# tusen-ai/SST

Measured on AMD Instinct MI355X. Metric: LiDAR frames/sec (SST backbone fwd+bwd) at Waymo 0.32m voxels, higher is better.
Workload: dtype f32 (storage, accumulation, attention, LayerNorm, reductions: fp32; the dense products of the encoder layers from the EXACT three-way bf16 split of both fp32 operands, six bf16 MFMA products with fp32 accumulation - error vs float64 <= 2 x the fp32 matrix pipe's: tests/test_gpu_dense_f32x6.py)

## Files before the change

include/sst_amd.h:

```cpp
#ifndef SST_AMD_H
#define SST_AMD_H

#include <stdint.h>

#ifdef __cplusplus
extern "C" {
#endif

#define SST_OK 0
#define SST_ERR_ARG (-1)
#define SST_ERR_UNSUPPORTED (-2)
#define SST_ERR_KEYSPACE (-3)

typedef enum { SST_REDUCE_SUM = 0, SST_REDUCE_MEAN = 1, SST_REDUCE_MAX = 2 } sst_reduce_t;

const char* sst_version(void);

int sst_dynamic_voxelize_f32(const float* d_points, int64_t n, int64_t row_stride,
                             const float voxel_size[3], const float coors_range[6],
                             int32_t* d_coors, int64_t coors_stride, int coors_col0, int batch_idx,
                             void* stream);
void sst_dynamic_voxelize_grid(const float voxel_size[3], const float coors_range[6], int32_t grid_xyz[3]);

int64_t sst_scan_workspace_bytes(int64_t n);
// ... 184 lines not shown
int sst_add_layernorm_act_bwd_f32(const float* d_dy, const float* d_sum, const float* d_stats, const float* d_weight,
                                  const float* d_bias, int act, int64_t m, int c, float* d_dx, float* d_dweight,
                                  float* d_dbias, void* d_workspace, void* stream);
int sst_add_layernorm_fwd_f32(const float* d_x, const float* d_res, const float* d_weight, const float* d_bias,
                              int64_t m, int c, float eps, float* d_y, float* d_sum, float* d_stats,
                              void* stream);
int sst_add_layernorm_pos_fwd_f32(const float* d_x, const float* d_res, const float* d_weight, const float* d_bias, int64_t m,
                                  int c, float eps, float* d_y, float* d_sum, float* d_stats, const float* d_pos_table,
                                  const int32_t* d_pos_idx, float* d_y_plus_pos, void* stream);
int64_t sst_add_layernorm_bwd_workspace_bytes(int64_t m, int c);
int sst_add_layernorm_bwd_f32(const float* d_dy, const float* d_sum, const float* d_stats,
                              const float* d_weight, int64_t m, int c, float* d_dx, float* d_dweight,
                              float* d_dbias, void* d_workspace, void* stream);
int64_t sst_colsum_workspace_bytes(int64_t m, int c);
int sst_colsum_f32(const float* d_x, int64_t m, int c, int64_t ld, float* d_out, void* d_workspace, void* stream);

int64_t sst_weight_grad_workspace_bytes(int64_t m, int out, int in);
int sst_weight_grad_f32(const float* d_dy, const float* d_x, int64_t m, int out, int in, int64_t ld_dy,
                        int64_t ld_x, float* d_dw, float* d_db, void* d_workspace, void* stream);
typedef struct sst_wgrad_problem_f32 {
  const float* dy;
  const float* x;
  int64_t m, ld_dy, ld_x;
  float* dw;
  float* db;
  int32_t out, in;
  const float* x_add_rows;
  const int32_t* x_add_index;
} sst_wgrad_problem_f32;
int64_t sst_weight_grad_group_workspace_bytes(const sst_wgrad_problem_f32* problems, int n);
int sst_weight_grad_group_f32(const sst_wgrad_problem_f32* problems, int n, void* d_workspace, void* stream);
int64_t sst_weight_grad_group_f32x6_workspace_bytes(const sst_wgrad_problem_f32* problems, int n);
int sst_weight_grad_group_f32x6(const sst_wgrad_problem_f32* problems, int n, void* d_workspace, void* stream);

int64_t sst_bn_workspace_bytes(int64_t n, int c);
int sst_bn_stats_f32(const float* d_x, int64_t n, int c, int64_t ld, float* d_mean, float* d_var,
                     void* d_workspace, void* stream);
int sst_bn_act_fwd_f32(const float* d_x, int64_t n, int c, int64_t ldx, const float* d_scale,
                       const float* d_shift, int act, float* d_y, int64_t ldy, void* stream);
int sst_bn_act_bwd_reduce_f32(const float* d_dy, const float* d_x, int64_t n, int c, int64_t lddy, int64_t ldx,
                              const float* d_mean, const float* d_invstd, const float* d_scale,
                              const float* d_shift, int act, float* d_sum_g, float* d_sum_gxhat,
                              void* d_workspace, void* stream);
int sst_bn_act_bwd_apply_f32(const float* d_dy, const float* d_x, int64_t n, int c, int64_t lddy, int64_t ldx,
                             const float* d_mean, const float* d_invstd, const float* d_scale,
                             const float* d_shift, const float* d_coef_a, const float* d_coef_b, float coef_scale,
                             int act, float* d_dx, int64_t lddx, void* stream);
int sst_bn_prepare_f32(const float* d_x, int64_t n, int c, int64_t ld, const float* d_weight, const float* d_bias,
                       float eps, float* d_running_mean, float* d_running_var, float factor, float* d_out4,
                       void* d_workspace, void* stream);
int sst_bn_prepare_tracked_f32(const float* d_x, int64_t n, int c, int64_t ld, const float* d_weight,
                               const float* d_bias, float eps, float* d_running_mean, float* d_running_var,
                               float factor, int64_t* d_num_batches_tracked, float* d_out4, void* d_workspace,
                               void* stream);
int sst_vfe_linear_moments_f32(const float* d_x, int64_t ldx, int64_t n, int k, const float* d_w, int64_t ldw, int c,
                               float* d_y, int64_t ldy, void* d_workspace, void* stream);
int sst_bn_prepare_from_partials_f32(int64_t n, int c, const float* d_weight, const float* d_bias, float eps,
                                     float* d_running_mean, float* d_running_var, float factor,
                                     int64_t* d_num_batches_tracked, float* d_out4, void* d_workspace, void* stream);
int sst_bn_stats_from_partials_f32(int64_t n, int c, float* d_mean, float* d_var, void* d_workspace, void* stream);
int sst_bn_act_pool_bwd_reduce_f32(const float* d_dy, const float* d_x, int64_t n, int c, int64_t lddy, int64_t ldx,
                                   const float* d_mean, const float* d_invstd, const float* d_scale, const float* d_shift,
                                   int act, const int32_t* d_group, const int32_t* d_arg, const float* d_dpool, int64_t ldp,
                                   float* d_sum_g, float* d_sum_gxhat, void* d_workspace, void* stream);
int sst_bn_act_pool_bwd_apply_f32(const float* d_dy, const float* d_x, int64_t n, int c, int64_t lddy, int64_t ldx,
                                  const float* d_mean, const float* d_invstd, const float* d_scale, const float* d_shift,
// ... 387 lines not shown
```

sst_amd/_lib.py:

```python
import ctypes
import os
import subprocess

import torch

_HERE = os.path.dirname(os.path.abspath(__file__))
_CSRC = os.path.join(_HERE, 'csrc')
LIB_PATH = os.path.join(_CSRC, 'libsst_amd.so')

_lib = None

c_i64 = ctypes.c_int64
c_i32 = ctypes.c_int
c_f32 = ctypes.c_float
c_ptr = ctypes.c_void_p



class WgradProblemBF16(ctypes.Structure):
    _fields_ = [('a', c_ptr), ('b', c_ptr), ('lda', c_i64), ('ldb', c_i64), ('m', c_i64), ('out_w', c_ptr),
                ('out_b', c_ptr), ('p', ctypes.c_int32), ('bias_side', ctypes.c_int32),
                ('transpose_out', ctypes.c_int32), ('reserved', ctypes.c_int32)]


# ... 137 lines not shown
    'sst_sra_attn_fwd_ord_f32': (c_i32, [c_ptr, c_ptr, c_ptr, c_i64, c_i64, c_i64, c_ptr, c_ptr, c_ptr, c_i64, c_i32,
                                         c_f32, c_i32, c_i32, c_ptr, c_i64, c_ptr, c_ptr]),
    'sst_sra_attn_bwd_ord_f32': (c_i32, [c_ptr] * 6 + [c_i64] * 5 + [c_ptr, c_ptr, c_ptr, c_i64, c_i64, c_i32, c_f32,
                                                                     c_i32, c_i32, c_ptr, c_ptr, c_ptr,
                                                                     c_i64, c_i64, c_i64, c_ptr, c_ptr]),
    'sst_sra_attn_bwd_workspace_bytes': (c_i64, [c_i64, c_i32]),
    'sst_sra_attn_cos_fwd_f32': (c_i32, [c_ptr, c_ptr, c_ptr, c_i64, c_i64, c_i64, c_ptr, c_ptr, c_ptr, c_i64, c_i32,
                                         c_ptr, c_i32, c_ptr, c_i64, c_ptr, c_ptr]),
    'sst_sra_attn_cos_bwd_f32': (c_i32, [c_ptr] * 6 + [c_i64] * 5 + [c_ptr, c_ptr, c_ptr, c_i64, c_i64, c_i32, c_ptr,
                                                                     c_i32, c_ptr, c_ptr, c_ptr,
                                                                     c_i64, c_i64, c_i64, c_ptr, c_ptr]),
    'sst_sra_attn_fwd_bf16': (c_i32, [c_ptr, c_ptr, c_ptr, c_i64, c_i64, c_i64, c_ptr, c_ptr, c_i64, c_i32, c_f32, c_i32,
                                      c_ptr, c_i64, c_ptr, c_ptr]),
    'sst_sra_attn_bwd_bf16': (c_i32, [c_ptr] * 6 + [c_i64] * 5 + [c_ptr, c_ptr, c_i64, c_i32, c_f32, c_i32, c_ptr, c_ptr,
                                                                  c_ptr, c_i64, c_i64, c_i64, c_ptr]),
    'sst_sra_attn_bf16_profile_next': (c_i32, [c_i32, c_ptr, c_ptr]),
    'sst_sra_attn_fwd_ord_bf16': (c_i32, [c_ptr, c_ptr, c_ptr, c_i64, c_i64, c_i64, c_ptr, c_ptr, c_ptr, c_i64, c_i32, c_f32,
                                          c_i32, c_ptr, c_i64, c_ptr, c_ptr]),
    'sst_sra_attn_bwd_ord_bf16': (c_i32, [c_ptr] * 6 + [c_i64] * 5 + [c_ptr, c_ptr, c_ptr, c_i64, c_i32, c_f32, c_i32, c_ptr,
                                                                      c_ptr, c_ptr, c_i64, c_i64, c_i64, c_ptr]),
    'sst_sra_attn_cos_fwd_bf16': (c_i32, [c_ptr, c_ptr, c_ptr, c_i64, c_i64, c_i64, c_ptr, c_ptr, c_ptr, c_i64, c_i32, c_ptr,
                                          c_i32, c_ptr, c_i64, c_ptr, c_ptr]),
    'sst_sra_attn_cos_bwd_bf16': (c_i32, [c_ptr] * 6 + [c_i64] * 5 + [c_ptr, c_ptr, c_ptr, c_i64, c_i32, c_ptr, c_i32, c_ptr,
                                                                      c_ptr, c_ptr, c_i64, c_i64, c_i64, c_ptr, c_ptr]),
    'sst_add_layernorm_fwd_bf16': (c_i32, [c_ptr, c_ptr, c_ptr, c_ptr, c_i64, c_i32, c_f32, c_ptr, c_ptr, c_ptr, c_ptr,
                                           c_ptr, c_ptr, c_ptr]),
    'sst_add_layernorm_bwd_bf16': (c_i32, [c_ptr, c_ptr, c_ptr, c_ptr, c_ptr, c_i64, c_i32, c_ptr, c_ptr, c_ptr, c_ptr,
                                           c_ptr]),
    'sst_cast_add_pos_bf16': (c_i32, [c_ptr, c_i32, c_i64, c_i32, c_ptr, c_ptr, c_ptr, c_ptr]),
    'sst_weight_grad_group_workspace_bytes': (c_i64, [c_ptr, c_i32]),
    'sst_weight_grad_group_f32': (c_i32, [c_ptr, c_i32, c_ptr, c_ptr]),
    'sst_weight_grad_group_f32x6_workspace_bytes': (c_i64, [c_ptr, c_i32]),
    'sst_weight_grad_group_f32x6': (c_i32, [c_ptr, c_i32, c_ptr, c_ptr]),
    'sst_tall_linear_ln_f32': (c_i32, [c_ptr, c_i64, c_ptr, c_i64, c_ptr, c_i64, c_i32, c_ptr, c_i64, c_ptr, c_ptr, c_f32, c_ptr,
                                       c_ptr, c_ptr, c_ptr, c_ptr, c_ptr, c_ptr]),
    'sst_tall_linear_ln_f32x3': (c_i32, [c_ptr, c_i64, c_ptr, c_i64, c_ptr, c_i64, c_i32, c_ptr, c_i64, c_ptr, c_ptr, c_f32, c_ptr,
                                         c_ptr, c_ptr, c_ptr, c_ptr, c_ptr, c_ptr]),
    'sst_tall_linear_epi_f32x3': (c_i32, [c_ptr, c_i64, c_ptr, c_i64, c_i32, c_ptr, c_i64, c_i32, c_i32, c_i32, c_ptr, c_ptr,
                                          c_i64, c_ptr, c_i64, c_ptr]),
    'sst_tall_linear_ln_f32x6': (c_i32, [c_ptr, c_i64, c_ptr, c_i64, c_ptr, c_i64, c_i32, c_ptr, c_i64, c_ptr, c_ptr, c_f32, c_ptr,
                                         c_ptr, c_ptr, c_ptr, c_ptr, c_ptr, c_ptr]),
    'sst_tall_linear_epi_f32x6': (c_i32, [c_ptr, c_i64, c_ptr, c_i64, c_i32, c_ptr, c_i64, c_i32, c_i32, c_i32, c_ptr, c_ptr,
                                          c_i64, c_ptr, c_i64, c_ptr]),
    'sst_tall_linear_epi2_f32x6': (c_i32, [c_ptr, c_ptr, c_i32, c_i64, c_ptr, c_i64, c_i32, c_ptr, c_i64, c_i32, c_i32, c_i32,
                                           c_ptr, c_ptr, c_i64, c_ptr, c_i64, c_ptr]),
    'sst_add_layernorm_bwd2_f32': (c_i32, [c_ptr, c_ptr, c_ptr, c_ptr, c_ptr, c_i64, c_i32, c_ptr, c_ptr, c_ptr, c_ptr, c_ptr]),
    'sst_tall_linear_epi_f32': (c_i32, [c_ptr, c_i64, c_ptr, c_i64, c_i32, c_ptr, c_i64, c_i32, c_i32, c_i32, c_ptr, c_ptr,
                                        c_i64, c_ptr, c_i64, c_ptr]),
    'sst_tall_linear_bf16': (c_i32, [c_ptr, c_i64, c_ptr, c_ptr, c_i64, c_i32, c_i32, c_i32, c_ptr, c_ptr, c_i64, c_ptr,
                                     c_i64, c_ptr]),
    'sst_tall_linear_ln_bf16': (c_i32, [c_ptr, c_i64, c_ptr, c_ptr, c_i64, c_i32, c_ptr, c_i64, c_ptr, c_ptr, c_f32, c_ptr, c_ptr,
                                        c_ptr, c_ptr, c_ptr, c_ptr, c_ptr]),
    'sst_wgrad_group_workspace_bytes': (c_i64, [c_ptr, c_i32]),
    'sst_wgrad_group_bf16': (c_i32, [c_ptr, c_i32, c_ptr, c_ptr]),
    'sst_cast_group_bf16': (c_i32, [c_ptr, c_i32, c_ptr]),
    'sst_gather_rows_f32': (c_i32, [c_ptr, c_i64, c_ptr, c_i64, c_i32, c_f32, c_ptr, c_i64, c_ptr]),
    'sst_add_table_rows_f32': (c_i32, [c_ptr, c_i64, c_ptr, c_i64, c_ptr, c_i64, c_i32, c_ptr, c_i64, c_ptr]),
    'sst_scatter_rows_f32': (c_i32, [c_ptr, c_i64, c_ptr, c_i64, c_i32, c_ptr, c_i64, c_ptr]),
    'sst_add_layernorm_fwd_f32': (c_i32, [c_ptr, c_ptr, c_ptr, c_ptr, c_i64, c_i32, c_f32, c_ptr, c_ptr, c_ptr,
                                          c_ptr]),
    'sst_add_layernorm_bwd_workspace_bytes': (c_i64, [c_i64, c_i32]),
    'sst_add_layernorm_pos_fwd_f32': (c_i32, [c_ptr, c_ptr, c_ptr, c_ptr, c_i64, c_i32, c_f32, c_ptr, c_ptr, c_ptr, c_ptr, c_ptr,
                                              c_ptr, c_ptr]),
    'sst_add_layernorm_act_fwd_f32': (c_i32, [c_ptr, c_ptr, c_ptr, c_ptr, c_i64, c_i32, c_f32, c_i32, c_ptr, c_ptr, c_ptr,
                                              c_ptr]),
    'sst_add_layernorm_act_bwd_f32': (c_i32, [c_ptr, c_ptr, c_ptr, c_ptr, c_ptr, c_i32, c_i64, c_i32, c_ptr, c_ptr, c_ptr,
# ... 256 lines not shown
```

sst_amd/csrc/layer_tail_x6.hip:

```cpp
#include <math.h>
#include <stdlib.h>
#include "common.h"

#ifndef SST_NT_OUT
#define SST_NT_OUT false
#endif
#ifndef SST_NT_BWD
#define SST_NT_BWD true
#endif

namespace {

typedef float f32x4 __attribute__((ext_vector_type(4)));
typedef float f32x2 __attribute__((ext_vector_type(2)));
typedef unsigned u32x4 __attribute__((ext_vector_type(4)));
typedef __bf16 bf16x8 __attribute__((ext_vector_type(8)));
typedef __bf16 bf16x2 __attribute__((ext_vector_type(2)));

__device__ __forceinline__ unsigned pack2(float lo, float hi) {
  const f32x2 v = {lo, hi};
  return __builtin_bit_cast(unsigned, __builtin_convertvector(v, bf16x2));
}
__device__ __forceinline__ float lo_f(unsigned p) { return __uint_as_float(p << 16); }
__device__ __forceinline__ float hi_f(unsigned p) { return __uint_as_float(p & 0xffff0000u); }
// ... 257 lines not shown
}

template <int HALF>
__device__ __forceinline__ void mma_half(const unsigned char* slot, int lane_off, const f32x4 (&x)[4][2], f32x4 (&acc)[8]) {
#pragma unroll
  for (int s2 = 0; s2 < 2; ++s2) {
    const img3 xs = split8(x[2 * HALF + s2][0], x[2 * HALF + s2][1]);
#pragma unroll
    for (int t0 = 0; t0 < 8; t0 += 4) {
      u32x4 a0[4], a1[4], a2[4];
#pragma unroll
      for (int u = 0; u < 4; ++u) {
        const int off = lane_off + ((t0 + u) * 2 + s2) * kFrag;
        a0[u] = *(const u32x4*)(slot + off);
        a1[u] = *(const u32x4*)(slot + kIA + off);
        a2[u] = *(const u32x4*)(slot + 2 * kIA + off);
      }
#pragma unroll
      for (int u = 0; u < 4; ++u) acc[t0 + u] = mma32(a0[u], xs.p2, acc[t0 + u]);
#pragma unroll
      for (int u = 0; u < 4; ++u) acc[t0 + u] = mma32(a2[u], xs.p0, acc[t0 + u]);
#pragma unroll
      for (int u = 0; u < 4; ++u) acc[t0 + u] = mma32(a1[u], xs.p1, acc[t0 + u]);
#pragma unroll
      for (int u = 0; u < 4; ++u) acc[t0 + u] = mma32(a0[u], xs.p1, acc[t0 + u]);
#pragma unroll
      for (int u = 0; u < 4; ++u) acc[t0 + u] = mma32(a1[u], xs.p0, acc[t0 + u]);
#pragma unroll
      for (int u = 0; u < 4; ++u) acc[t0 + u] = mma32(a0[u], xs.p0, acc[t0 + u]);
    }
  }
}

__device__ __forceinline__ void mma_first(const unsigned char* slot, int lane_off1, const img3 (&y)[4], f32x4& out0, f32x4& out1) {
  const f32x4 z = {0.f, 0.f, 0.f, 0.f};
  f32x4 am[2] = {z, z}, ca[2] = {z, z}, cb[2] = {z, z};
#pragma unroll
  for (int s = 0; s < 4; ++s) {
    u32x4 a0[2], a1[2], a2[2];
#pragma unroll
    for (int T = 0; T < 2; ++T) {
      const int off = lane_off1 + (T * 4 + s) * kFrag;
      a0[T] = *(const u32x4*)(slot + off);
      a1[T] = *(const u32x4*)(slot + kI1 + off);
      a2[T] = *(const u32x4*)(slot + 2 * kI1 + off);
    }
#pragma unroll
    for (int T = 0; T < 2; ++T) ca[T] = mma32(a0[T], y[s].p2, ca[T]);
#pragma unroll
    for (int T = 0; T < 2; ++T) cb[T] = mma32(a0[T], y[s].p1, cb[T]);
#pragma unroll
    for (int T = 0; T < 2; ++T) ca[T] = mma32(a2[T], y[s].p0, ca[T]);
#pragma unroll
    for (int T = 0; T < 2; ++T) am[T] = mma32(a0[T], y[s].p0, am[T]);
#pragma unroll
    for (int T = 0; T < 2; ++T) ca[T] = mma32(a1[T], y[s].p1, ca[T]);
#pragma unroll
    for (int T = 0; T < 2; ++T) cb[T] = mma32(a1[T], y[s].p0, cb[T]);
  }
  out0 = am[0] + (cb[0] + ca[0]);
  out1 = am[1] + (cb[1] + ca[1]);
}

__device__ __forceinline__ void mma_second(const unsigned char* slot2, int lane_off2, const img3& h, f32x4 (&acc)[8]) {
#pragma unroll
  for (int t0 = 0; t0 < 8; t0 += 4) {
    u32x4 a0[4], a1[4], a2[4];
#pragma unroll
    for (int u = 0; u < 4; ++u) {
      const int off = lane_off2 + (t0 + u) * kFrag;
      a0[u] = *(const u32x4*)(slot2 + off);
      a1[u] = *(const u32x4*)(slot2 + kI2 + off);
      a2[u] = *(const u32x4*)(slot2 + 2 * kI2 + off);
    }
#pragma unroll
    for (int u = 0; u < 4; ++u) acc[t0 + u] = mma32(a0[u], h.p2, acc[t0 + u]);
#pragma unroll
    for (int u = 0; u < 4; ++u) acc[t0 + u] = mma32(a2[u], h.p0, acc[t0 + u]);
#pragma unroll
    for (int u = 0; u < 4; ++u) acc[t0 + u] = mma32(a1[u], h.p1, acc[t0 + u]);
#pragma unroll
    for (int u = 0; u < 4; ++u) acc[t0 + u] = mma32(a0[u], h.p1, acc[t0 + u]);
#pragma unroll
    for (int u = 0; u < 4; ++u) acc[t0 + u] = mma32(a1[u], h.p0, acc[t0 + u]);
#pragma unroll
    for (int u = 0; u < 4; ++u) acc[t0 + u] = mma32(a0[u], h.p0, acc[t0 + u]);
  }
}

__device__ __forceinline__ void ln_stats(f32x4 (&v)[4][2], float eps, float& mean, float& rstd) {
  float sum = 0.f;
#pragma unroll
  for (int s = 0; s < 4; ++s)
#pragma unroll
// ... 81 lines not shown
    f32x4 v[4][2];
#pragma unroll
    for (int s = 0; s < 4; ++s) {
      const int n0 = 32 * s + 8 * g;
      v[s][0] = acc[2 * s] + *(const f32x4*)(par + n0) + xr[s][0];
      v[s][1] = acc[2 * s + 1] + *(const f32x4*)(par + n0 + 4) + xr[s][1];
      if (P.s1 != nullptr) store32<true>(io, P.s1, kC, 32 * s, v[s][0], v[s][1]);
    }
    float mean, rstd;
    ln_stats(v, P.eps, mean, rstd);
    if (valid && g == 0) ((float2*)P.st1)[row] = make_float2(mean, rstd);
#pragma unroll
    for (int s = 0; s < 4; ++s) {
      const int n0 = 32 * s + 8 * g;
      const f32x4 y0 = v[s][0] * rstd * *(const f32x4*)(par + kC + n0) + *(const f32x4*)(par + 2 * kC + n0);
      const f32x4 y1 = v[s][1] * rstd * *(const f32x4*)(par + kC + n0 + 4) + *(const f32x4*)(par + 2 * kC + n0 + 4);
      store32<true>(io, P.y1, kC, 32 * s, y0, y1);
      yi[s] = split8(y0, y1);
    }
#pragma unroll
    for (int T = 0; T < 8; ++T) acc[T] = z4;
  }
  barrier_drain();
  f32x4 sp0 = z4, sp1 = z4, sh0 = z4, sh1 = z4;
#pragma unroll 1
  for (int j = 0; j < kNF; ++j) {
    if (j > 0) {
      store32<true>(io, P.pre, kFF, kHC * (j - 1), sp0, sp1);
      store32<true>(io, P.h, kFF, kHC * (j - 1), sh0, sh1);
    }
    f32x4 p0, p1;
    mma_first(lds, lane_off1, yi, p0, p1);
    const int nl = kHC * j + 8 * g;
    p0 += *(const f32x4*)(par + 6 * kC + nl);
    p1 += *(const f32x4*)(par + 6 * kC + nl + 4);
    f32x4 h0, h1;
#pragma unroll
    for (int r = 0; r < 4; ++r) {
      h0[r] = ACT == 1 ? gelu_f(p0[r]) : fmaxf(p0[r], 0.f);
      h1[r] = ACT == 1 ? gelu_f(p1[r]) : fmaxf(p1[r], 0.f);
    }
    const img3 hs = split8(h0, h1);
    barrier_drain();
    if (j + 1 < kNF) dma_pieces(packed + (size_t)(j + 3) * kSlot, lds, kPart1 / 1024, wave, lane);
    mma_second(part2, lane_off2, hs, acc);
    sp0 = p0, sp1 = p1, sh0 = h0, sh1 = h1;
    barrier_drain();
    if (j + 1 < kNF) dma_pieces(packed + (size_t)(j + 3) * kSlot + kPart1, part2, kPart2 / 1024, wave, lane);
  }
  store32<true>(io, P.pre, kFF, kHC * (kNF - 1), sp0, sp1);
  store32<true>(io, P.h, kFF, kHC * (kNF - 1), sh0, sh1);
  f32x4 v[4][2];
#pragma unroll
  for (int s = 0; s < 4; ++s) {
    const int n0 = 32 * s + 8 * g;
    f32x4 ya, yb;
    join8(yi[s], ya, yb);
    v[s][0] = acc[2 * s] + *(const f32x4*)(par + 3 * kC + n0) + ya;
    v[s][1] = acc[2 * s + 1] + *(const f32x4*)(par + 3 * kC + n0 + 4) + yb;
    if (P.s2 != nullptr) store32<true>(io, P.s2, kC, 32 * s, v[s][0], v[s][1]);
  }
  float mean, rstd;
  ln_stats(v, P.eps, mean, rstd);
  if (valid && g == 0) ((float2*)P.st2)[row] = make_float2(mean, rstd);
  const float* prow = P.pos_table != nullptr ? P.pos_table + (size_t)P.pos_idx[row] * kC : nullptr;
#pragma unroll
  for (int s = 0; s < 4; ++s) {
    const int n0 = 32 * s + 8 * g;
// ... 352 lines not shown
```

sst_amd/csrc/wgrad_x6.hip:

```cpp
#include <math.h>
#include <stdlib.h>
#include "common.h"

namespace {

typedef float f32x4 __attribute__((ext_vector_type(4)));
typedef float f32x2 __attribute__((ext_vector_type(2)));
typedef unsigned u32x4 __attribute__((ext_vector_type(4)));
typedef unsigned u32x2 __attribute__((ext_vector_type(2)));
typedef __bf16 bf16x8 __attribute__((ext_vector_type(8)));
typedef __bf16 bf16x2 __attribute__((ext_vector_type(2)));

__device__ __forceinline__ unsigned pack2(float lo, float hi) {
  const f32x2 v = {lo, hi};
  return __builtin_bit_cast(unsigned, __builtin_convertvector(v, bf16x2));
}
__device__ __forceinline__ float lo_f(unsigned p) { return __uint_as_float(p << 16); }
__device__ __forceinline__ float hi_f(unsigned p) { return __uint_as_float(p & 0xffff0000u); }
__device__ __forceinline__ f32x4 mma32(u32x4 a, u32x4 b, f32x4 c) {
  return __builtin_amdgcn_mfma_f32_16x16x32_bf16(__builtin_bit_cast(bf16x8, a), __builtin_bit_cast(bf16x8, b), c, 0, 0, 0);
}
__device__ __forceinline__ void split2(float a, float b, unsigned& p0, unsigned& p1, unsigned& p2) {
  p0 = pack2(a, b);
  const float ra = a - lo_f(p0), rb = b - hi_f(p0);
  p1 = pack2(ra, rb);
  p2 = pack2(ra - lo_f(p1), rb - hi_f(p1));
}

constexpr int kMaxProblems = 8;
constexpr int kTile = 128;
constexpr int kStep = 32;
constexpr int kTileLds = 1040;
constexpr int kImage = 8 * kTileLds;
constexpr int kStage = 2 * 3 * kImage;
constexpr int kLdsBytes = 2 * kStage;

struct x6_problem {
  const float* dy;
  const float* x;
  int64_t m, ld_dy, ld_x;
  int out, in;
  int tile0;
  int db_off;
  float* dw;
  float* db;
  const float* x_add_rows;
  const int32_t* x_add_index;
};
struct x6_group {
  x6_problem p[kMaxProblems];
  int n, tiles, slices;
  int64_t tokens_per_slice;
};

__global__ __launch_bounds__(512, 2) void wgrad_x6_k(const x6_group G, float* __restrict__ part, float* __restrict__ dbp) {
  extern __shared__ __attribute__((aligned(16))) unsigned char lds[];
  const int tid = threadIdx.x, lane = tid & 63, wave = tid >> 6;
  const int l15 = lane & 15, g = lane >> 4;
  const int tile = blockIdx.x / G.slices, slice = blockIdx.x - tile * G.slices;
  int pi = 0;
#pragma unroll
  for (int q = 1; q < kMaxProblems; ++q)
    if (q < G.n && tile >= G.p[q].tile0) pi = q;
  const x6_problem P = G.p[pi];
  const int tiles_k = P.in / kTile;
  const int tl = tile - P.tile0, tn = tl / tiles_k, tk = tl - tn * tiles_k;
  const int n0 = tn * kTile, k0 = tk * kTile;
  const int64_t t_begin = (int64_t)slice * G.tokens_per_slice;
  int64_t t_end = t_begin + G.tokens_per_slice;
  t_end = t_end < P.m ? t_end : P.m;

  const int op = tid >> 8, tq = (tid >> 5) & 7, cg = tid & 31;
  const float* src = op == 0 ? P.dy + n0 + 4 * cg : P.x + k0 + 4 * cg;
  const int64_t ld = op == 0 ? P.ld_dy : P.ld_x;
  const int st_off = (cg >> 2) * kTileLds + (tq & 1) * 512 + (tq >> 1) * 128 + (cg & 3) * 32;
  constexpr int kPf = 2;
  f32x4 rows[kPf][4];
  const int64_t t_last = t_end > 0 ? t_end - 1 : 0;
  const bool xadd = op == 1 && P.x_add_rows != nullptr;
  const float* addsrc = xadd ? P.x_add_rows + k0 + 4 * cg : nullptr;
  f32x4 prow[kPf][4];
  int32_t pidx[4] = {0, 0, 0, 0};
  auto load_idx = [&](int64_t t0) {
#pragma unroll
    for (int r = 0; r < 4; ++r) {
      int64_t t = t0 + 4 * tq + r;
      t = t < t_last ? t : t_last;
      pidx[r] = P.x_add_index[t];
    }
  };
  auto load_rows = [&](int64_t t0, f32x4 (&dst)[4], f32x4 (&pdst)[4]) {
#pragma unroll
    for (int r = 0; r < 4; ++r) {
      int64_t t = t0 + 4 * tq + r;
      t = t < t_last ? t : t_last;
      dst[r] = *(const f32x4*)(src + t * ld);
    }
    if (xadd) {
#pragma unroll
      for (int r = 0; r < 4; ++r) pdst[r] = *(const f32x4*)(addsrc + (int64_t)pidx[r] * P.in);
      load_idx(t0 + kStep);
    }
  };
  float bsum[4] = {0.f, 0.f, 0.f, 0.f};
  u32x4 img[3][2];
  auto split_col = [&](int e, int64_t t0, const f32x4 (&rws)[4], const f32x4 (&prw)[4]) {
    float v[4];
#pragma unroll
    for (int r = 0; r < 4; ++r) v[r] = (t0 + 4 * tq + r < t_end) ? (xadd ? rws[r][e] + prw[r][e] : rws[r][e]) : 0.f;
    if (op == 0) bsum[e] += (v[0] + v[1]) + (v[2] + v[3]);
    unsigned a0, a1, a2, b0, b1, b2;
    split2(v[0], v[1], a0, a1, a2);
    split2(v[2], v[3], b0, b1, b2);
    img[0][e >> 1][2 * (e & 1)] = a0;
    img[0][e >> 1][2 * (e & 1) + 1] = b0;
    img[1][e >> 1][2 * (e & 1)] = a1;
    img[1][e >> 1][2 * (e & 1) + 1] = b1;
    img[2][e >> 1][2 * (e & 1)] = a2;
    img[2][e >> 1][2 * (e & 1) + 1] = b2;
  };
  auto store_img = [&](int buf) {
    unsigned char* base = lds + buf * kStage + op * 3 * kImage + st_off;
#pragma unroll
    for (int im = 0; im < 3; ++im) {
      *(u32x4*)(base + im * kImage) = img[im][0];
      *(u32x4*)(base + im * kImage + 16) = img[im][1];
    }
  };
  const int wn = wave & 3, wk = wave >> 2;
  const int frag_off = g * 128 + l15 * 8;
  f32x4 acc[4][2], acl[4][2];
#pragma unroll
  for (int a = 0; a < 4; ++a)
#pragma unroll
    for (int b = 0; b < 2; ++b) acc[a][b] = acl[a][b] = (f32x4){0.f, 0.f, 0.f, 0.f};
  auto frag = [&](const unsigned char* image, int tile16) -> u32x4 {
    const unsigned char* p = image + tile16 * kTileLds + frag_off;
    const u32x2 lo = *(const u32x2*)p, hi = *(const u32x2*)(p + 512);
    return (u32x4){lo[0], lo[1], hi[0], hi[1]};
  };

  if (xadd) load_idx(t_begin);
#pragma unroll
  for (int u = 0; u < kPf; ++u) load_rows(t_begin + (int64_t)u * kStep, rows[u], prow[u]);
#pragma unroll
  for (int e = 0; e < 4; ++e) split_col(e, t_begin, rows[0], prow[0]);
  store_img(0);
  load_rows(t_begin + (int64_t)kPf * kStep, rows[0], prow[0]);
  __syncthreads();
  const int64_t n_steps = (t_end - t_begin + kStep - 1) / kStep;
  for (int64_t s0 = 0; s0 < n_steps; s0 += kPf) {
#pragma unroll
    for (int u = 0; u < kPf; ++u) {
      const int64_t s = s0 + u;
      if (s >= n_steps) break;
      const int64_t t1 = t_begin + (s + 1) * kStep;
      const unsigned char* dyi = lds + (u & 1) * kStage;
      const unsigned char* xi = dyi + 3 * kImage;
      u32x4 b0[2], b1[2], b2[2];
#pragma unroll
      for (int b = 0; b < 2; ++b) {
        b0[b] = frag(dyi, 2 * wn + b);
        b1[b] = frag(dyi + kImage, 2 * wn + b);
        b2[b] = frag(dyi + 2 * kImage, 2 * wn + b);
      }
#pragma unroll
      for (int a = 0; a < 4; ++a) {
        const u32x4 a0 = frag(xi, 4 * wk + a), a1 = frag(xi + kImage, 4 * wk + a), a2 = frag(xi + 2 * kImage, 4 * wk + a);
#pragma unroll
        for (int b = 0; b < 2; ++b) acl[a][b] = mma32(a2, b0[b], acl[a][b]);
#pragma unroll
        for (int b = 0; b < 2; ++b) acl[a][b] = mma32(a0, b2[b], acl[a][b]);
#pragma unroll
        for (int b = 0; b < 2; ++b) acl[a][b] = mma32(a1, b1[b], acl[a][b]);
#pragma unroll
        for (int b = 0; b < 2; ++b) acl[a][b] = mma32(a1, b0[b], acl[a][b]);
#pragma unroll
        for (int b = 0; b < 2; ++b) acl[a][b] = mma32(a0, b1[b], acl[a][b]);
#pragma unroll
        for (int b = 0; b < 2; ++b) acc[a][b] = mma32(a0, b0[b], acc[a][b]);
        split_col(a, t1, rows[(u + 1) % kPf], prow[(u + 1) % kPf]);
      }
      store_img((u + 1) & 1);
      load_rows(t1 + (int64_t)kPf * kStep, rows[(u + 1) % kPf], prow[(u + 1) % kPf]);
      __syncthreads();
    }
  }
#pragma unroll
  for (int a = 0; a < 4; ++a)
#pragma unroll
    for (int b = 0; b < 2; ++b) acc[a][b] += acl[a][b];
  float* dst = part + ((int64_t)tile * G.slices + slice) * (kTile * kTile);
#pragma unroll
  for (int a = 0; a < 4; ++a)
#pragma unroll
    for (int b = 0; b < 2; ++b)
      *(f32x4*)(dst + (32 * wn + 16 * b + l15) * kTile + 64 * wk + 16 * a + 4 * g) = acc[a][b];
  if (P.db_off >= 0 && tk == 0) {
    float* red = (float*)lds;
    if (op == 0) *(f32x4*)(red + tq * 128 + 4 * cg) = (f32x4){bsum[0], bsum[1], bsum[2], bsum[3]};
    __syncthreads();
    if (tid < 128) {
      float s = 0.f;
#pragma unroll
      for (int q = 0; q < 8; ++q) s += red[q * 128 + tid];
      dbp[((int64_t)P.db_off + n0 + tid) * G.slices + slice] = s;
    }
  }
}

struct x6_riders {
  sst_colsum_rider r[2];
  int n, blocks0;
};

constexpr int kRedQuads = 32, kRedGroups = 8;

__global__ __launch_bounds__(256) void wgrad_x6_reduce_k(const x6_group G, const float* __restrict__ part,
// ... 100 lines not shown
  x6_group& G = plan->g;
  G.n = n;
  int tiles = 0, db_cols = 0;
  int64_t m = pr[0].m;
  for (int i = 0; i < n; ++i) {
    const sst_wgrad_problem_f32& p = pr[i];
    if (p.m != m || p.m < 1 || p.out < kTile || p.in < kTile || (p.out % kTile) || (p.in % kTile) || (p.ld_dy & 3) ||
        (p.ld_x & 3) || !p.dy || !p.x || !p.dw || !aligned16(p.dy) || !aligned16(p.x) || !aligned16(p.dw))
      return false;
    G.p[i].dy = p.dy;
    G.p[i].x = p.x;
    G.p[i].m = p.m;
    G.p[i].ld_dy = p.ld_dy;
    G.p[i].ld_x = p.ld_x;
    G.p[i].out = p.out;
    G.p[i].in = p.in;
    G.p[i].tile0 = tiles;
    G.p[i].db_off = p.db ? db_cols : -1;
    G.p[i].dw = p.dw;
    G.p[i].db = p.db;
    if ((p.x_add_rows != nullptr) != (p.x_add_index != nullptr) || (p.x_add_rows && !aligned16(p.x_add_rows))) return false;
    G.p[i].x_add_rows = p.x_add_rows;
    G.p[i].x_add_index = p.x_add_index;
    tiles += (p.out / kTile) * (p.in / kTile);
    if (p.db) db_cols += p.out;
  }
  G.tiles = tiles;
  int slices = (256 / tiles) & ~7;
  if (slices < 8) slices = 8;
  const int64_t max_slices = sst_div_up(m, (int64_t)kStep);
  while (slices > 8 && slices > max_slices) slices -= 8;
  G.slices = slices;
  G.tokens_per_slice = sst_align_up(sst_div_up(m, (int64_t)slices), (int64_t)kStep);
  plan->part_bytes = sst_align_up((int64_t)tiles * slices * kTile * kTile * 4, 256);
  plan->db_bytes = sst_align_up((int64_t)(db_cols > 0 ? db_cols : 1) * slices * 4, 256);
  return true;
}

}

extern "C" {

int64_t sst_weight_grad_group_f32x6_workspace_bytes(const sst_wgrad_problem_f32* problems, int n) {
  x6_plan plan;
  if (!make_plan(problems, n, &plan)) return SST_ERR_UNSUPPORTED;
  return plan.part_bytes + plan.db_bytes;
}

}

int sst_internal_weight_grad_group_f32x6(const sst_wgrad_problem_f32* problems, int n, void* d_workspace,
                                         const sst_colsum_rider* riders, int n_riders, void* stream) {
  x6_plan plan;
  if (!make_plan(problems, n, &plan)) return SST_ERR_UNSUPPORTED;
  if (!d_workspace || !aligned16(d_workspace)) return SST_ERR_ARG;
  hipStream_t st = (hipStream_t)stream;
  float* part = (float*)d_workspace;
  float* dbp = (float*)((char*)d_workspace + plan.part_bytes);
  static unsigned long long configured = 0;
  if (sst_first_use_on_device(&configured)) {
    SST_HIP(hipFuncSetAttribute((const void*)wgrad_x6_k, hipFuncAttributeMaxDynamicSharedMemorySize, kLdsBytes));
    sst_mark_device(&configured);
  }
  const int64_t quads = (int64_t)plan.g.tiles * (kTile * kTile / 4);
  const int tile_blocks = (int)sst_div_up(quads, (int64_t)kRedQuads);
  if (n_riders < 0 || n_riders > 2 || (n_riders > 0 && !riders)) return SST_ERR_ARG;
  x6_riders R;
  R.n = n_riders, R.blocks0 = 0;
  int extra = 0;
  for (int i = 0; i < n_riders; ++i) {
    const sst_colsum_rider& q = riders[i];
    if (!q.partials || q.nb < 1 || q.width < 1 || !q.out0 || !q.out1) return SST_ERR_ARG;
    R.r[i] = q;
    if (i == 0) R.blocks0 = (q.width + 31) / 32;
    extra += (q.width + 31) / 32;
  }
  hipLaunchKernelGGL(wgrad_x6_k, dim3((unsigned)(plan.g.tiles * plan.g.slices)), dim3(512), kLdsBytes, st, plan.g, part, dbp);
  hipLaunchKernelGGL(wgrad_x6_reduce_k, dim3((unsigned)(tile_blocks + extra)), dim3(256), 0, st, plan.g, part, dbp, extra, R);
  SST_LAUNCH_CHECK();
// ... 11 lines not shown
```

Measured before the change: 99.06.

## Add lean unmasked steady-state loop to f32x6 weight-grad kernel with scalar addressing

Splits the weight-grad x6 main loop into a lean phase for slices whose tokens are fully in range and a checked tail phase. The lean phase drops per-row bounds masks and uses wave-uniform 64-bit bases (readfirstlane) plus 32-bit per-lane offsets, which cuts VALU address arithmetic and masking. Bias summation is restricted to the blocks that actually need it, and masking and x_add are hoisted out of the per-column split. A plan query entry point is exported for inspection. The cost is more code and an ld < 2^24 guard that falls back to the old path.

```diff
diff --git a/include/sst_amd.h b/include/sst_amd.h
--- a/include/sst_amd.h
+++ b/include/sst_amd.h
@@ -240,6 +240,8 @@
 int sst_weight_grad_group_f32(const sst_wgrad_problem_f32* problems, int n, void* d_workspace, void* stream);
 int64_t sst_weight_grad_group_f32x6_workspace_bytes(const sst_wgrad_problem_f32* problems, int n);
 int sst_weight_grad_group_f32x6(const sst_wgrad_problem_f32* problems, int n, void* d_workspace, void* stream);
+int sst_weight_grad_group_f32x6_plan(const sst_wgrad_problem_f32* problems, int n, int* tiles, int* slices,
+                                     int64_t* tokens_per_slice, int* lean_slices);
 
 int64_t sst_bn_workspace_bytes(int64_t n, int c);
 int sst_bn_stats_f32(const float* d_x, int64_t n, int c, int64_t ld, float* d_mean, float* d_var,
diff --git a/sst_amd/_lib.py b/sst_amd/_lib.py
--- a/sst_amd/_lib.py
+++ b/sst_amd/_lib.py
@@ -193,6 +193,7 @@
     'sst_weight_grad_group_f32': (c_i32, [c_ptr, c_i32, c_ptr, c_ptr]),
     'sst_weight_grad_group_f32x6_workspace_bytes': (c_i64, [c_ptr, c_i32]),
     'sst_weight_grad_group_f32x6': (c_i32, [c_ptr, c_i32, c_ptr, c_ptr]),
+    'sst_weight_grad_group_f32x6_plan': (c_i32, [c_ptr, c_i32, c_ptr, c_ptr, c_ptr, c_ptr]),
     'sst_tall_linear_ln_f32': (c_i32, [c_ptr, c_i64, c_ptr, c_i64, c_ptr, c_i64, c_i32, c_ptr, c_i64, c_ptr, c_ptr, c_f32, c_ptr,
                                        c_ptr, c_ptr, c_ptr, c_ptr, c_ptr, c_ptr]),
     'sst_tall_linear_ln_f32x3': (c_i32, [c_ptr, c_i64, c_ptr, c_i64, c_ptr, c_i64, c_i32, c_ptr, c_i64, c_ptr, c_ptr, c_f32, c_ptr,
diff --git a/sst_amd/csrc/layer_tail_x6.hip b/sst_amd/csrc/layer_tail_x6.hip
--- a/sst_amd/csrc/layer_tail_x6.hip
+++ b/sst_amd/csrc/layer_tail_x6.hip
@@ -313,6 +313,10 @@
   }
 }
 
+__device__ __forceinline__ f32x4 add4(const f32x4& a, const f32x4& b) {
+  return (f32x4){a[0] + b[0], a[1] + b[1], a[2] + b[2], a[3] + b[3]};
+}
+
 __device__ __forceinline__ void mma_first(const unsigned char* slot, int lane_off1, const img3 (&y)[4], f32x4& out0, f32x4& out1) {
   const f32x4 z = {0.f, 0.f, 0.f, 0.f};
   f32x4 am[2] = {z, z}, ca[2] = {z, z}, cb[2] = {z, z};
@@ -339,8 +343,8 @@
 #pragma unroll
     for (int T = 0; T < 2; ++T) cb[T] = mma32(a1[T], y[s].p0, cb[T]);
   }
-  out0 = am[0] + (cb[0] + ca[0]);
-  out1 = am[1] + (cb[1] + ca[1]);
+  out0 = add4(am[0], add4(cb[0], ca[0]));
+  out1 = add4(am[1], add4(cb[1], ca[1]));
 }
 
 __device__ __forceinline__ void mma_second(const unsigned char* slot2, int lane_off2, const img3& h, f32x4 (&acc)[8]) {
@@ -488,8 +492,8 @@
     f32x4 p0, p1;
     mma_first(lds, lane_off1, yi, p0, p1);
     const int nl = kHC * j + 8 * g;
-    p0 += *(const f32x4*)(par + 6 * kC + nl);
-    p1 += *(const f32x4*)(par + 6 * kC + nl + 4);
+    p0 = add4(p0, *(const f32x4*)(par + 6 * kC + nl));
+    p1 = add4(p1, *(const f32x4*)(par + 6 * kC + nl + 4));
     f32x4 h0, h1;
 #pragma unroll
     for (int r = 0; r < 4; ++r) {
diff --git a/sst_amd/csrc/wgrad_x6.hip b/sst_amd/csrc/wgrad_x6.hip
--- a/sst_amd/csrc/wgrad_x6.hip
+++ b/sst_amd/csrc/wgrad_x6.hip
@@ -1,5 +1,6 @@
 #include <math.h>
 #include <stdlib.h>
+#include <type_traits>
 #include "common.h"
 
 namespace {
@@ -27,9 +28,18 @@
   p2 = pack2(ra - lo_f(p1), rb - hi_f(p1));
 }
 
+__device__ __forceinline__ int64_t uniform64(int64_t v) {
+  const unsigned lo = __builtin_amdgcn_readfirstlane((unsigned)(uint64_t)v);
+  const unsigned hi = __builtin_amdgcn_readfirstlane((unsigned)((uint64_t)v >> 32));
+  return (int64_t)(((uint64_t)hi << 32) | lo);
+}
+
+typedef const __attribute__((address_space(1))) char* gbytes;
+
 constexpr int kMaxProblems = 8;
 constexpr int kTile = 128;
 constexpr int kStep = 32;
+constexpr int kPf = 2;
 constexpr int kTileLds = 1040;
 constexpr int kImage = 8 * kTileLds;
 constexpr int kStage = 2 * 3 * kImage;
@@ -50,6 +60,7 @@
 struct x6_group {
   x6_problem p[kMaxProblems];
   int n, tiles, slices;
+  int lean_slices;
   int64_t tokens_per_slice;
 };
 
@@ -57,7 +68,7 @@
   extern __shared__ __attribute__((aligned(16))) unsigned char lds[];
   const int tid = threadIdx.x, lane = tid & 63, wave = tid >> 6;
   const int l15 = lane & 15, g = lane >> 4;
-  const int tile = blockIdx.x / G.slices, slice = blockIdx.x - tile * G.slices;
+  const int tile = __builtin_amdgcn_readfirstlane(blockIdx.x / G.slices), slice = blockIdx.x - tile * G.slices;
   int pi = 0;
 #pragma unroll
   for (int q = 1; q < kMaxProblems; ++q)
@@ -70,14 +81,14 @@
   int64_t t_end = t_begin + G.tokens_per_slice;
   t_end = t_end < P.m ? t_end : P.m;
 
-  const int op = tid >> 8, tq = (tid >> 5) & 7, cg = tid & 31;
+  const int op = __builtin_amdgcn_readfirstlane(tid >> 8), tq = (tid >> 5) & 7, cg = tid & 31;
   const float* src = op == 0 ? P.dy + n0 + 4 * cg : P.x + k0 + 4 * cg;
   const int64_t ld = op == 0 ? P.ld_dy : P.ld_x;
   const int st_off = (cg >> 2) * kTileLds + (tq & 1) * 512 + (tq >> 1) * 128 + (cg & 3) * 32;
-  constexpr int kPf = 2;
   f32x4 rows[kPf][4];
   const int64_t t_last = t_end > 0 ? t_end - 1 : 0;
   const bool xadd = op == 1 && P.x_add_rows != nullptr;
+  const bool bias = op == 0 && P.db_off >= 0 && tk == 0;
   const float* addsrc = xadd ? P.x_add_rows + k0 + 4 * cg : nullptr;
   f32x4 prow[kPf][4];
   int32_t pidx[4] = {0, 0, 0, 0};
@@ -102,16 +113,55 @@
       load_idx(t0 + kStep);
     }
   };
+  const int64_t lean_ld4 = uniform64(ld * 4);
+  const gbytes lean_src = (gbytes)uniform64((int64_t)(op == 0 ? P.dy + n0 : P.x + k0)) + uniform64(t_begin) * lean_ld4;
+  const gbytes lean_idx = (gbytes)uniform64((int64_t)(P.x_add_index + t_begin));
+  unsigned lean_off[4];
+#pragma unroll
+  for (int r = 0; r < 4; ++r) lean_off[r] = ((unsigned)(4 * tq + r) * (unsigned)ld + 4u * cg) * 4u;
+  unsigned lean_ioff = 16u * tq;
+  auto load_rows_lean = [&](int64_t s, f32x4 (&dst)[4], f32x4 (&pdst)[4]) {
+    const gbytes base = lean_src + s * kStep * lean_ld4;
+#pragma unroll
+    for (int r = 0; r < 4; ++r) {
+      asm volatile("" : "+v"(lean_off[r]));
+      dst[r] = *(const __attribute__((address_space(1))) f32x4*)(base + lean_off[r]);
+    }
+    if (xadd) {
+#pragma unroll
+      for (int r = 0; r < 4; ++r) pdst[r] = *(const f32x4*)((const char*)addsrc + (int64_t)pidx[r] * (int64_t)(4 * P.in));
+      const gbytes ib = lean_idx + (s + 1) * kStep * 4;
+      asm volatile("" : "+v"(lean_ioff));
+#pragma unroll
+      for (int r = 0; r < 4; ++r) pidx[r] = *(const __attribute__((address_space(1))) int32_t*)(ib + lean_ioff + 4 * r);
+    }
+  };
   float bsum[4] = {0.f, 0.f, 0.f, 0.f};
+  auto finish_rows = [&](auto lean, int64_t t0, f32x4 (&rws)[4], const f32x4 (&prw)[4]) {
+    if (xadd) {
+#pragma unroll
+      for (int r = 0; r < 4; ++r)
+#pragma unroll
+        for (int e = 0; e < 4; ++e) rws[r][e] = rws[r][e] + prw[r][e];
+    }
+    if constexpr (!decltype(lean)::value) {
+#pragma unroll
+      for (int r = 0; r < 4; ++r) {
+        const bool in = t0 + 4 * tq + r < t_end;
+#pragma unroll
+        for (int e = 0; e < 4; ++e) rws[r][e] = in ? rws[r][e] : 0.f;
+      }
+    }
+    if (bias) {
+#pragma unroll
+      for (int e = 0; e < 4; ++e) bsum[e] += (rws[0][e] + rws[1][e]) + (rws[2][e] + rws[3][e]);
+    }
+  };
   u32x4 img[3][2];
-  auto split_col = [&](int e, int64_t t0, const f32x4 (&rws)[4], const f32x4 (&prw)[4]) {
-    float v[4];
-#pragma unroll
-    for (int r = 0; r < 4; ++r) v[r] = (t0 + 4 * tq + r < t_end) ? (xadd ? rws[r][e] + prw[r][e] : rws[r][e]) : 0.f;
-    if (op == 0) bsum[e] += (v[0] + v[1]) + (v[2] + v[3]);
+  auto split_col = [&](int e, const f32x4 (&rws)[4]) {
     unsigned a0, a1, a2, b0, b1, b2;
-    split2(v[0], v[1], a0, a1, a2);
-    split2(v[2], v[3], b0, b1, b2);
+    split2(rws[0][e], rws[1][e], a0, a1, a2);
+    split2(rws[2][e], rws[3][e], b0, b1, b2);
     img[0][e >> 1][2 * (e & 1)] = a0;
     img[0][e >> 1][2 * (e & 1) + 1] = b0;
     img[1][e >> 1][2 * (e & 1)] = a1;
@@ -143,47 +193,61 @@
   if (xadd) load_idx(t_begin);
 #pragma unroll
   for (int u = 0; u < kPf; ++u) load_rows(t_begin + (int64_t)u * kStep, rows[u], prow[u]);
-#pragma unroll
-  for (int e = 0; e < 4; ++e) split_col(e, t_begin, rows[0], prow[0]);
+  finish_rows(std::false_type{}, t_begin, rows[0], prow[0]);
+#pragma unroll
+  for (int e = 0; e < 4; ++e) split_col(e, rows[0]);
   store_img(0);
   load_rows(t_begin + (int64_t)kPf * kStep, rows[0], prow[0]);
   __syncthreads();
+  auto step = [&](auto lean, int u, int64_t s) {
+    const int64_t t1 = t_begin + (s + 1) * kStep;
+    f32x4(&rws)[4] = rows[(u + 1) % kPf];
+    f32x4(&prw)[4] = prow[(u + 1) % kPf];
+    finish_rows(lean, t1, rws, prw);
+    const unsigned char* dyi = lds + (u & 1) * kStage;
+    const unsigned char* xi = dyi + 3 * kImage;
+    u32x4 b0[2], b1[2], b2[2];
+#pragma unroll
+    for (int b = 0; b < 2; ++b) {
+      b0[b] = frag(dyi, 2 * wn + b);
+      b1[b] = frag(dyi + kImage, 2 * wn + b);
+      b2[b] = frag(dyi + 2 * kImage, 2 * wn + b);
+    }
+#pragma unroll
+    for (int a = 0; a < 4; ++a) {
+      const u32x4 a0 = frag(xi, 4 * wk + a), a1 = frag(xi + kImage, 4 * wk + a), a2 = frag(xi + 2 * kImage, 4 * wk + a);
+#pragma unroll
+      for (int b = 0; b < 2; ++b) acl[a][b] = mma32(a2, b0[b], acl[a][b]);
+#pragma unroll
+      for (int b = 0; b < 2; ++b) acl[a][b] = mma32(a0, b2[b], acl[a][b]);
+#pragma unroll
+      for (int b = 0; b < 2; ++b) acl[a][b] = mma32(a1, b1[b], acl[a][b]);
+#pragma unroll
+      for (int b = 0; b < 2; ++b) acl[a][b] = mma32(a1, b0[b], acl[a][b]);
+#pragma unroll
+      for (int b = 0; b < 2; ++b) acl[a][b] = mma32(a0, b1[b], acl[a][b]);
+#pragma unroll
+      for (int b = 0; b < 2; ++b) acc[a][b] = mma32(a0, b0[b], acc[a][b]);
+      split_col(a, rws);
+    }
+    store_img((u + 1) & 1);
+    if constexpr (decltype(lean)::value)
+      load_rows_lean(s + 1 + kPf, rws, prw);
+    else
+      load_rows(t1 + (int64_t)kPf * kStep, rws, prw);
+    __syncthreads();
+  };
   const int64_t n_steps = (t_end - t_begin + kStep - 1) / kStep;
-  for (int64_t s0 = 0; s0 < n_steps; s0 += kPf) {
+  const int64_t s_lean = uniform64(slice < G.lean_slices ? ((n_steps - 1) / kPf) * kPf : 0);
+  for (int64_t s0 = 0; s0 < s_lean; s0 += kPf) {
+#pragma unroll
+    for (int u = 0; u < kPf; ++u) step(std::true_type{}, u, s0 + u);
+  }
+  for (int64_t s0 = s_lean; s0 < n_steps; s0 += kPf) {
 #pragma unroll
     for (int u = 0; u < kPf; ++u) {
-      const int64_t s = s0 + u;
-      if (s >= n_steps) break;
-      const int64_t t1 = t_begin + (s + 1) * kStep;
-      const unsigned char* dyi = lds + (u & 1) * kStage;
-      const unsigned char* xi = dyi + 3 * kImage;
-      u32x4 b0[2], b1[2], b2[2];
-#pragma unroll
-      for (int b = 0; b < 2; ++b) {
-        b0[b] = frag(dyi, 2 * wn + b);
-        b1[b] = frag(dyi + kImage, 2 * wn + b);
-        b2[b] = frag(dyi + 2 * kImage, 2 * wn + b);
-      }
-#pragma unroll
-      for (int a = 0; a < 4; ++a) {
-        const u32x4 a0 = frag(xi, 4 * wk + a), a1 = frag(xi + kImage, 4 * wk + a), a2 = frag(xi + 2 * kImage, 4 * wk + a);
-#pragma unroll
-        for (int b = 0; b < 2; ++b) acl[a][b] = mma32(a2, b0[b], acl[a][b]);
-#pragma unroll
-        for (int b = 0; b < 2; ++b) acl[a][b] = mma32(a0, b2[b], acl[a][b]);
-#pragma unroll
-        for (int b = 0; b < 2; ++b) acl[a][b] = mma32(a1, b1[b], acl[a][b]);
-#pragma unroll
-        for (int b = 0; b < 2; ++b) acl[a][b] = mma32(a1, b0[b], acl[a][b]);
-#pragma unroll
-        for (int b = 0; b < 2; ++b) acl[a][b] = mma32(a0, b1[b], acl[a][b]);
-#pragma unroll
-        for (int b = 0; b < 2; ++b) acc[a][b] = mma32(a0, b0[b], acc[a][b]);
-        split_col(a, t1, rows[(u + 1) % kPf], prow[(u + 1) % kPf]);
-      }
-      store_img((u + 1) & 1);
-      load_rows(t1 + (int64_t)kPf * kStep, rows[(u + 1) % kPf], prow[(u + 1) % kPf]);
-      __syncthreads();
+      if (s0 + u >= n_steps) break;
+      step(std::false_type{}, u, s0 + u);
     }
   }
 #pragma unroll
@@ -350,6 +414,12 @@
   while (slices > 8 && slices > max_slices) slices -= 8;
   G.slices = slices;
   G.tokens_per_slice = sst_align_up(sst_div_up(m, (int64_t)slices), (int64_t)kStep);
+  int64_t lean = (m - (int64_t)(kPf + 2) * kStep) / G.tokens_per_slice;
+  lean = lean < 0 ? 0 : (lean > slices ? slices : lean);
+  if (G.tokens_per_slice < 3 * kStep) lean = 0;
+  for (int i = 0; i < n; ++i)
+    if (pr[i].ld_dy < 0 || pr[i].ld_x < 0 || pr[i].ld_dy >= (1 << 24) || pr[i].ld_x >= (1 << 24)) lean = 0;
+  G.lean_slices = (int)lean;
   plan->part_bytes = sst_align_up((int64_t)tiles * slices * kTile * kTile * 4, 256);
   plan->db_bytes = sst_align_up((int64_t)(db_cols > 0 ? db_cols : 1) * slices * 4, 256);
   return true;
@@ -363,6 +433,17 @@
   x6_plan plan;
   if (!make_plan(problems, n, &plan)) return SST_ERR_UNSUPPORTED;
   return plan.part_bytes + plan.db_bytes;
+}
+
+int sst_weight_grad_group_f32x6_plan(const sst_wgrad_problem_f32* problems, int n, int* tiles, int* slices,
+                                     int64_t* tokens_per_slice, int* lean_slices) {
+  x6_plan plan;
+  if (!make_plan(problems, n, &plan)) return SST_ERR_UNSUPPORTED;
+  if (tiles) *tiles = plan.g.tiles;
+  if (slices) *slices = plan.g.slices;
+  if (tokens_per_slice) *tokens_per_slice = plan.g.tokens_per_slice;
+  if (lean_slices) *lean_slices = plan.g.lean_slices;
+  return SST_OK;
 }
 
 }
```

Measured after the change: 101.8, median of 6. +2.8%, better.
